# tranqkhue/bugcar_image_segmentation

Measured on AMD Instinct MI355X. Metric: frames/sec ENet 640x480 segmentation -> BEV occupancy grid (synthetic), whole job, higher is better.
Workload: dtype fp32; 1 GPU; config3/5: ENet 640x480 batch 64 per GPU, preprocess + forward + argmax/LUT + fused BEV warp/occgrid (1000x1000 BEV -> 200x200 cells); global_batch=64, per_gpu_batch=64, height=480, width=640, parallelism=frame-sharded dp1, streams_per_gpu=1, hip_graph=True, ranks=1, devices=1, backend=none (one process)

## Files before the change

### bugcar_image_segmentation_amd/build.py

```python
from __future__ import annotations

import os
import subprocess
import sys
from concurrent.futures import ThreadPoolExecutor
from pathlib import Path

PKG = Path(__file__).resolve().parent
ROOT = PKG.parent
CSRC = PKG / "csrc"
OBJ = PKG / "_build"
LIB = PKG / "libbugseg.so"
SOURCES = ["conv_kernels.hip", "cls_kernels.hip", "init_kernels.hip", "bneck_kernels.hip", "bneck2_kernels.hip", "up_kernels.hip", "prep_kernels.hip",
           "bev_kernels.hip", "deeplab_kernels.hip", "road_kernels.hip", "clahe_kernels.hip", "canny_kernels.hip", "eval_kernels.hip", "hough_kernels.hip", "quad_kernels.hip", "bugseg_runtime.cpp", "deeplab_runtime.cpp"]
HEADERS = [CSRC / "bneck_pair_kernels.hip", CSRC / "bugseg_internal.h", CSRC / "deeplab_internal.h", CSRC / "knobs.h", CSRC / "mfma_common.h", CSRC / "cls_common.h", CSRC / "ccl_common.h", ROOT / "include" / "bugseg.h"]
ARCH = os.environ.get("BUGSEG_OFFLOAD_ARCH", "gfx950")
SOURCE_FLAGS = {"cls_kernels.hip": ["-mllvm", "-amdgpu-mfma-vgpr-form=1"], "clahe_kernels.hip": ["-ffp-contract=off"],
                "hough_kernels.hip": ["-ffp-contract=off"], "quad_kernels.hip": ["-ffp-contract=off"]}


def _hipcc() -> str:
    for c in (os.environ.get("HIPCC"), "/opt/rocm/bin/hipcc", "hipcc"):
        if c and (os.path.sep not in c or os.path.exists(c)):
            return c
    raise RuntimeError("hipcc not found")


def _stale(target: Path, deps) -> bool:
    if not target.exists():
        return True
    t = target.stat().st_mtime
    return any(Path(d).stat().st_mtime > t for d in deps)


def build_native(force: bool = False, verbose: bool = False, stamps: bool = False, variant: str = "",
                 defines=()) -> Path:
    if stamps:
        variant, defines = "stamps", ("-DBUGSEG_STAMPS", *defines)
    obj_dir = OBJ / variant if variant else OBJ
    lib = PKG / f"libbugseg_{variant}.so" if variant else LIB
    obj_dir.mkdir(parents=True, exist_ok=True)
    hipcc = _hipcc()
    flags = [f"--offload-arch={ARCH}", "-O3", "-std=c++17", "-fPIC", "-Wall", "-Wno-unused-function",
             f"-I{ROOT / 'include'}", f"-I{CSRC}", *defines]
    jobs = []
    for s in SOURCES:
        src = CSRC / s
        obj = obj_dir / (s + ".o")
        if force or _stale(obj, [src, *HEADERS]):
            lang = ["-x", "hip"] if s.endswith(".hip") else []
            jobs.append((obj, [hipcc, *flags, *SOURCE_FLAGS.get(s, []), *lang, "-c", str(src), "-o", str(obj)]))

    def run(job):
        obj, cmd = job
        if verbose:
            print(" ".join(cmd), file=sys.stderr)
        r = subprocess.run(cmd, capture_output=True, text=True)
        if r.returncode != 0:
            raise RuntimeError(f"compile failed: {' '.join(cmd)}\n{r.stdout}\n{r.stderr}")
        return obj

    with ThreadPoolExecutor(max_workers=min(4, max(1, len(jobs)))) as ex:
        list(ex.map(run, jobs))
    objs = [obj_dir / (s + ".o") for s in SOURCES]
    if force or jobs or _stale(lib, objs):
        tmp = lib.with_suffix(".so.tmp")
        cmd = [hipcc, f"--offload-arch={ARCH}", "-shared", "-fPIC", "-o", str(tmp), *map(str, objs)]
        r = subprocess.run(cmd, capture_output=True, text=True)
        if r.returncode != 0:
            raise RuntimeError(f"link failed: {' '.join(cmd)}\n{r.stdout}\n{r.stderr}")
        os.replace(tmp, lib)
    return lib


if __name__ == "__main__":
    var = next((a.split("=", 1)[1] for a in sys.argv if a.startswith("--variant=")), "")
    print(build_native(force="--force" in sys.argv, verbose=True, stamps="--stamps" in sys.argv, variant=var,
                       defines=tuple(a for a in sys.argv if a.startswith("-D"))))
```

### bugcar_image_segmentation_amd/csrc/bneck_pair_kernels.hip

```cpp
#include <algorithm>

#include "bugseg_internal.h"
#include "mfma_common.h"

namespace bugseg {

namespace {
constexpr int PC = 64, PKS1 = 2, PKS2 = 5, PG2 = 18, PNR3 = 4;
constexpr int PK1S = PKS1 * 32 + 8, PK2S = PKS2 * 32 + 8, PK3S = 32 + 8;
constexpr int PW1 = 16 * PK1S, PW2 = 16 * PK2S, PW3 = PC * PK3S;
constexpr int PWF = PW1 + PW2 + PW3;
constexpr int PCST = 4 * 16 + 3 * PC;
constexpr int PBLK = PWF + PCST;
constexpr int PZP = 8;
#ifndef BNECK_PAIR_YSTR
#define BNECK_PAIR_YSTR 68
#endif
constexpr int PYS = BNECK_PAIR_YSTR;
static_assert(PYS >= PC && PYS % 4 == 0, "a y pixel is 64 floats, 16-B aligned");

template <int TH, int NW>
struct PairForm {
    static constexpr int TW = 16, NT = NW * 64;
    static constexpr int HWA = TW + 4, HRA = (TH + 4) * HWA;
    static constexpr int HWB = TW + 2, HRB = (TH + 2) * HWB;
    static constexpr int NFA = (HRA + 15) / 16, NFB = (HRB + 15) / 16;
    static constexpr int NCA = (NFA + NW - 1) / NW, NCB = (NFB + NW - 1) / NW, NCT = (TH + NW - 1) / NW;
    static constexpr int ZPAD = 2 * PBLK, Y = ZPAD + PZP, T0 = Y + HRB * PYS;
    static constexpr int PLOA = HRA * 8, PLOB = HRB * 8;
    static constexpr int END = T0 + 2 * PLOA;
    static constexpr size_t LDS_BYTES = (size_t)END * 4;
    static_assert(Y % 4 == 0 && T0 % 4 == 0, "every region starts on a 16-B boundary");
    static_assert(NW <= 2 * PLOA, "the range maxima fit in the t0 region");
    static_assert(LDS_BYTES <= 160 * 1024, "a CU has 160 KB of LDS");
};

__device__ __forceinline__ void ldw_hl(RawS &r, const float *p, int kq) {
    r.h = *reinterpret_cast<const uint4 *>(p + kq * 4);
    r.l = *reinterpret_cast<const uint4 *>(p + 16 + kq * 4);
}
__device__ __forceinline__ void st4pl(float *t0, int plo, int h, int ch, float4 v) {
    const float e[4] = {v.x, v.y, v.z, v.w};
    _Float16 hh[4], ll[4];
#pragma unroll
    for (int i = 0; i < 4; ++i) {
        hh[i] = (_Float16)e[i];
        ll[i] = (_Float16)(e[i] - (float)hh[i]);
    }
    unsigned char *b = reinterpret_cast<unsigned char *>(t0 + h * 8) + (ch >> 3) * 16 + (ch & 7) * 2;
    *reinterpret_cast<f16x4 *>(b) = (f16x4){hh[0], hh[1], hh[2], hh[3]};
    *reinterpret_cast<f16x4 *>(b + plo * 4) = (f16x4){ll[0], ll[1], ll[2], ll[3]};
}
}

template <int TH, int NW>
__global__ void __launch_bounds__(NW * 64, 1) bneck_pair_kernel(const BneckPairArgs p) {
    using F = PairForm<TH, NW>;
    constexpr int TW = F::TW, HWA = F::HWA, HRA = F::HRA, HWB = F::HWB, HRB = F::HRB;
    extern __shared__ __attribute__((aligned(16))) float psm[];
    const BneckArgs &a = p.a, &b = p.b;
    span_enter(a.span);
    const int grp = (int)(blockIdx.x & 7), slot = (int)(blockIdx.x >> 3), nslots = (int)(gridDim.x >> 3);
    const int CH = tile_walk_ch(a.ntiles);
    if (tile_walk(grp, slot, CH, a.ntiles, a.rev) < 0) {
        span_exit(a.span);
        return;
    }
    const int tid = threadIdx.x, lane = tid & 63, col = lane & 15, kq = lane >> 4;
    const int wave = __builtin_amdgcn_readfirstlane(tid >> 6);
    const float rl = rng_lane(a.rg);
#pragma unroll
    for (int k = 0; k < 2; ++k) {
        const BneckArgs &q = k ? b : a;
        float *base_k = psm + k * PBLK;
        constexpr int SR1 = PK1S / 4, SR2 = PK2S / 4, SR3 = PK3S / 4, CPR1 = PKS1 * 8, CPR2 = PKS2 * 8, CPR3 = 8;
        constexpr int S1 = 16 * SR1, S2 = 16 * SR2, NSL = PWF / 4;
        static_assert(NSL % 64 == 0, "whole wave instructions");
        for (int base = wave * 64; base < NSL; base += F::NT) {
            const int s = base + lane;
            const uint4 *src;
            auto pick = [&](const void *w, int i, int SR, int CPR) {
                const int r = i / SR, c = i - r * SR;
                const int cs = (c & ~7) | ((c & 7) < 4 ? 2 * (c & 7) : 2 * (c & 3) + 1);
                src = (const uint4 *)w + r * CPR + (c < CPR ? cs : 0);
            };
            if (s < S1) pick(q.w1, s, SR1, CPR1);
            else if (s < S1 + S2) pick(q.w2, s - S1, SR2, CPR2);
            else pick(q.w3, s - S1 - S2, SR3, CPR3);
            __builtin_amdgcn_global_load_lds((__attribute__((address_space(1))) void *)src,
                                             (__attribute__((address_space(3))) void *)(base_k + (size_t)base * 4), 16, 0, 0);
        }
        float *cb1 = base_k + PWF, *cs1 = cb1 + 16, *cb2 = cs1 + 16, *cs2 = cb2 + 16, *cb3 = cs2 + 16, *cs3 = cb3 + PC, *cso = cs3 + PC;
        if (tid < 16) { cb1[tid] = q.b1[tid]; cs1[tid] = q.s1[tid]; cb2[tid] = q.b2[tid]; cs2[tid] = q.s2[tid]; }
        if (tid < PC) { cb3[tid] = q.b3[tid]; cs3[tid] = q.s3[tid]; cso[tid] = q.s_out[tid]; }
    }
    if (tid < PZP) psm[F::ZPAD + tid] = 0.f;
    asm volatile("s_waitcnt vmcnt(0)" ::: "memory");
    if (bneck_range<false>(a.rg, rng_reduce(rl)).any) {
        span_exit(a.span);
        return;
    }
    __syncthreads();

    float *const zpad = psm + F::ZPAD, *const ys = psm + F::Y, *const t0 = psm + F::T0;
    const auto rxb = mkbuf(a.x, a.x_bytes);
    const auto rob = mkbuf(b.out, a.x_bytes);
    auto act = [](float4 v, const float *s) { return prelu4m(v, ld4f(s)); };
    const float4 zero4 = make_float4(0.f, 0.f, 0.f, 0.f);
    float amy = 0.f, amo = 0.f;

    auto blk = [&](int k, const float *&w1, const float *&w2, const float *&w3, const float *&cb1) {
        w1 = psm + k * PBLK; w2 = w1 + PW1; w3 = w2 + PW2; cb1 = w3 + PW3;
    };
    auto project = [&](const float *w1, const float *cb1, const RawF (&xs)[PKS1]) -> float4 {
        f32x4 acc = bias4(cb1 + kq * 4);
#pragma unroll
        for (int s = 0; s < PKS1; ++s) {
            RawS wf;
            ldw_hl(wf, w1 + col * PK1S + s * 32, kq);
            mma(acc, wf, xs[s]);
        }
        return act(f4(acc), cb1 + 16 + kq * 4);
    };
    auto middle = [&](const float *w2, const float *cb2, int hc, int hw, int plo, RawF &tf) {
        f32x4 acc = bias4(cb2 + kq * 4);
#pragma unroll
        for (int s = 0; s < PKS2; ++s) {
            const int g = s * 4 + kq;
            const int tap = g >> 1, coff = (g & 1) * 4;
            const int ky = tap / 3, kx = tap - ky * 3;
            int off = (hc + ky * hw + kx) * 8 + coff;
            asm volatile("" : "+v"(off));
            RawS xf, wf;
            xf.h = *reinterpret_cast<const uint4 *>(g < PG2 ? t0 + off : zpad);
            xf.l = *reinterpret_cast<const uint4 *>(g < PG2 ? t0 + plo + off : zpad);
            ldw_hl(wf, w2 + col * PK2S + s * 32, kq);
            mma(acc, wf, xf);
        }
        to_bop(tf, act(f4(acc), cb2 + 16 + kq * 4), zero4);
    };
    auto expand = [&](const float *w3, const float *cb3, int r, const RawF &tf, float4 res) -> float4 {
        const int ch = r * 16 + kq * 4;
        f32x4 acc = bias4(cb3 + ch);
        RawS wf;
        ldw_hl(wf, w3 + (r * 16 + col) * PK3S, kq);
        mma(acc, wf, tf);
        const float4 v = act(f4(acc), cb3 + PC + ch);
        return act(add4(v, res), cb3 + 2 * PC + ch);
    };

    const int wword = tile_walk_mirror(grp, CH, a.ntiles, a.rev);
    for (int it = slot; it < CH; it += nslots) {
        int tile = grp * CH + it;
        if (tile >= a.ntiles) break;
        tile = tile_walk_flip(wword, tile);
        const int txi = tile % a.tiles_x, t2 = tile / a.tiles_x;
        const int tyi = t2 % a.tiles_y, n = t2 / a.tiles_y;
        const int oy0 = a.oy_base + tyi * TH, ox0 = txi * TW;
        const uint32_t xn = (uint32_t)(n * a.H * a.W) * (uint32_t)(PC * 4);
        auto pix = [&](int y, int x) -> uint32_t {
            uint32_t v = xn + (__umul24((uint32_t)y, (uint32_t)a.W) + (uint32_t)x) * (uint32_t)(PC * 4);
            asm volatile("" : "+v"(v));
            return (unsigned)y < (unsigned)a.H && (unsigned)x < (unsigned)a.W ? v : OOB;
        };
        const float *w1, *w2, *w3, *cb1;

        blk(0, w1, w2, w3, cb1);
        {
            RawF xf[F::NCA][PKS1];
            uint32_t po[F::NCA];
#pragma unroll
            for (int c = 0; c < F::NCA; ++c) {
                const int f = wave + NW * c;
                if (f >= F::NFA) break;
                const int h = f * 16 + col, hy = h / HWA, hx = h - hy * HWA;
                po[c] = h < HRA ? pix(oy0 - 2 + hy, ox0 - 2 + hx) : OOB;
#pragma unroll
                for (int s = 0; s < PKS1; ++s) bld8(xf[c][s], rxb, po[c] == OOB ? OOB : po[c] + (uint32_t)((s * 4 + kq) * 32));
            }
#pragma unroll
            for (int c = 0; c < F::NCA; ++c) {
                const int f = wave + NW * c;
                if (f >= F::NFA) break;
                const int h = f * 16 + col;
                float4 v = project(w1, cb1, xf[c]);
                if (po[c] == OOB) v = zero4;
                if (h < HRA) st4pl(t0, F::PLOA, h, kq * 4, v);
            }
        }
        __syncthreads();

#pragma unroll
        for (int c = 0; c < F::NCB; ++c) {
            const int f = wave + NW * c;
            if (f >= F::NFB) break;
            const int q = f * 16 + col, qq = q < HRB ? q : 0;
            const int ry = qq / HWB, rx = qq - ry * HWB;
            const uint32_t po = q < HRB ? pix(oy0 - 1 + ry, ox0 - 1 + rx) : OOB;
            uint4 res[PNR3];
#pragma unroll
            for (int r = 0; r < PNR3; ++r) res[r] = bld16(rxb, po == OOB ? OOB : po + (uint32_t)((r * 16 + kq * 4) * 4));
            RawF tf;
            middle(w2, cb1 + 32, ry * HWA + rx, HWA, F::PLOA, tf);
#pragma unroll
            for (int r = 0; r < PNR3; ++r) {
                float4 v = expand(w3, cb1 + 64, r, tf, __builtin_bit_cast(float4, res[r]));
                if (po == OOB) v = zero4;
                rng_acc4(amy, v);
                if (q < HRB) st4(ys + q * PYS + r * 16 + kq * 4, v);
            }
        }
        __syncthreads();

        blk(1, w1, w2, w3, cb1);
#pragma unroll
        for (int c = 0; c < F::NCB; ++c) {
            const int f = wave + NW * c;
            if (f >= F::NFB) break;
            const int q = f * 16 + col, qq = q < HRB ? q : 0;
            const int ry = qq / HWB, rx = qq - ry * HWB;
            const bool ok = q < HRB && (unsigned)(oy0 - 1 + ry) < (unsigned)a.H && (unsigned)(ox0 - 1 + rx) < (unsigned)a.W;
            RawF xs[PKS1];
#pragma unroll
            for (int s = 0; s < PKS1; ++s) ld8(xs[s], ys + qq * PYS + (s * 4 + kq) * 8);
            float4 v = project(w1, cb1, xs);
            if (!ok) v = zero4;
            if (q < HRB) st4pl(t0, F::PLOB, q, kq * 4, v);
        }
        __syncthreads();

#pragma unroll
        for (int c = 0; c < F::NCT; ++c) {
            const int f = wave + NW * c;
            if (f >= TH) break;
            RawF tf;
            middle(w2, cb1 + 32, f * HWB + col, HWB, F::PLOB, tf);
            const float *yr = ys + ((f + 1) * HWB + col + 1) * PYS;
            const uint32_t po = pix(oy0 + f, ox0 + col), po_o = pix(oy0 + f, ox0 + (col ^ 8));
            const bool lo8 = col < 8;
            const uint32_t pa = lo8 ? po : po_o, pb = lo8 ? po_o : po;
#pragma unroll
            for (int u = 0; u < PNR3 / 2; ++u) {
                float4 v2[2];
#pragma unroll
                for (int hh = 0; hh < 2; ++hh) {
                    const int r = 2 * u + hh;
                    v2[hh] = expand(w3, cb1 + 64, r, tf, ld4(yr + r * 16 + kq * 4));
                    rng_acc4(amo, v2[hh]);
                }
                const uint4 u0 = __builtin_bit_cast(uint4, v2[0]), u1 = __builtin_bit_cast(uint4, v2[1]);
                const uint4 xs = lo8 ? u1 : u0;
                uint4 yx;
                yx.x = (uint32_t)__builtin_amdgcn_update_dpp(0, (int)xs.x, 0x128, 0xf, 0xf, false);
                yx.y = (uint32_t)__builtin_amdgcn_update_dpp(0, (int)xs.y, 0x128, 0xf, 0xf, false);
                yx.z = (uint32_t)__builtin_amdgcn_update_dpp(0, (int)xs.z, 0x128, 0xf, 0xf, false);
                yx.w = (uint32_t)__builtin_amdgcn_update_dpp(0, (int)xs.w, 0x128, 0xf, 0xf, false);
                const uint32_t cb = (uint32_t)(u * 32 + (lo8 ? 0 : 16) + kq * 4) * 4u;
                bst16o<16>(rob, pa == OOB ? OOB : pa + cb, lo8 ? u0 : yx);
                bst16o<16>(rob, pb == OOB ? OOB : pb + cb, lo8 ? yx : u1);
            }
        }
        __syncthreads();
    }
    rng_commit_wg(amy, a.rg.amax_out, t0, NW);
    rng_commit_wg(amo, b.rg.amax_out, t0, NW);
    span_exit(a.span);
}

#ifndef BNECK_PAIR_TH
#define BNECK_PAIR_TH 12
#endif
#ifndef BNECK_PAIR_NW
#define BNECK_PAIR_NW 16
#endif
using PairBuilt = PairForm<BNECK_PAIR_TH, BNECK_PAIR_NW>;
static const void *pair_fun() { return (const void *)bneck_pair_kernel<BNECK_PAIR_TH, BNECK_PAIR_NW>; }

void bneck_pair_shape(int &th, int &tw, int &threads, size_t &lds) {
    th = BNECK_PAIR_TH; tw = PairBuilt::TW; threads = PairBuilt::NT; lds = PairBuilt::LDS_BYTES;
}

hipError_t launch_bneck_pair(const Knobs &k, const BneckPairArgs &a, hipStream_t s) {
    hipError_t e = allow_dynamic_lds(pair_fun());
    if (e != hipSuccess) return e;
    const int g = resident_grid(k, pair_fun(), PairBuilt::NT, PairBuilt::LDS_BYTES, a.a.ntiles);
    void *args[] = {const_cast<BneckPairArgs *>(&a)};
    return hipLaunchKernel(pair_fun(), dim3(g), dim3(PairBuilt::NT), args, PairBuilt::LDS_BYTES, s);
}

}
```

Baseline: 23560 frames/s.

## Prefetch next tile's input in bneck pair kernel and reuse staged input as residual

```diff
diff --git a/bugcar_image_segmentation_amd/build.py b/bugcar_image_segmentation_amd/build.py
--- a/bugcar_image_segmentation_amd/build.py
+++ b/bugcar_image_segmentation_amd/build.py
@@ -34,9 +34,13 @@
 
 
 def build_native(force: bool = False, verbose: bool = False, stamps: bool = False, variant: str = "",
-                 defines=()) -> Path:
+                 defines=(), only=()) -> Path:
     if stamps:
         variant, defines = "stamps", ("-DBUGSEG_STAMPS", *defines)
+    if not variant:
+        only = ()
+    if only:
+        build_native(verbose=verbose)
     obj_dir = OBJ / variant if variant else OBJ
     lib = PKG / f"libbugseg_{variant}.so" if variant else LIB
     obj_dir.mkdir(parents=True, exist_ok=True)
@@ -45,6 +49,8 @@
              f"-I{ROOT / 'include'}", f"-I{CSRC}", *defines]
     jobs = []
     for s in SOURCES:
+        if only and s not in only:
+            continue
         src = CSRC / s
         obj = obj_dir / (s + ".o")
         if force or _stale(obj, [src, *HEADERS]):
@@ -62,7 +68,7 @@
 
     with ThreadPoolExecutor(max_workers=min(4, max(1, len(jobs)))) as ex:
         list(ex.map(run, jobs))
-    objs = [obj_dir / (s + ".o") for s in SOURCES]
+    objs = [(obj_dir if not only or s in only else OBJ) / (s + ".o") for s in SOURCES]
     if force or jobs or _stale(lib, objs):
         tmp = lib.with_suffix(".so.tmp")
         cmd = [hipcc, f"--offload-arch={ARCH}", "-shared", "-fPIC", "-o", str(tmp), *map(str, objs)]
@@ -75,5 +81,6 @@
 
 if __name__ == "__main__":
     var = next((a.split("=", 1)[1] for a in sys.argv if a.startswith("--variant=")), "")
+    only = next((tuple(a.split("=", 1)[1].split(",")) for a in sys.argv if a.startswith("--only=")), ())
     print(build_native(force="--force" in sys.argv, verbose=True, stamps="--stamps" in sys.argv, variant=var,
-                       defines=tuple(a for a in sys.argv if a.startswith("-D"))))
+                       defines=tuple(a for a in sys.argv if a.startswith("-D")), only=only))
diff --git a/bugcar_image_segmentation_amd/csrc/bneck_pair_kernels.hip b/bugcar_image_segmentation_amd/csrc/bneck_pair_kernels.hip
--- a/bugcar_image_segmentation_amd/csrc/bneck_pair_kernels.hip
+++ b/bugcar_image_segmentation_amd/csrc/bneck_pair_kernels.hip
@@ -18,6 +18,19 @@
 #endif
 constexpr int PYS = BNECK_PAIR_YSTR;
 static_assert(PYS >= PC && PYS % 4 == 0, "a y pixel is 64 floats, 16-B aligned");
+#ifndef BNECK_PAIR_XLDS
+#define BNECK_PAIR_XLDS 1
+#endif
+#ifndef BNECK_PAIR_PREF
+#define BNECK_PAIR_PREF 1
+#endif
+#ifndef BNECK_PAIR_PREFAT
+#define BNECK_PAIR_PREFAT 2
+#endif
+#ifndef STAMP
+#define STAMP(k) do {} while (0)
+#define STAMP_WG() do {} while (0)
+#endif
 
 template <int TH, int NW>
 struct PairForm {
@@ -150,45 +163,76 @@
     };
 
     const int wword = tile_walk_mirror(grp, CH, a.ntiles, a.rev);
-    for (int it = slot; it < CH; it += nslots) {
-        int tile = grp * CH + it;
-        if (tile >= a.ntiles) break;
-        tile = tile_walk_flip(wword, tile);
+    auto tile_at = [&](int it) -> int {
+        const int tile = grp * CH + it;
+        return it < CH && tile < a.ntiles ? tile_walk_flip(wword, tile) : -1;
+    };
+    auto origin = [&](int tile, int &oy0, int &ox0, uint32_t &xn) {
         const int txi = tile % a.tiles_x, t2 = tile / a.tiles_x;
         const int tyi = t2 % a.tiles_y, n = t2 / a.tiles_y;
-        const int oy0 = a.oy_base + tyi * TH, ox0 = txi * TW;
-        const uint32_t xn = (uint32_t)(n * a.H * a.W) * (uint32_t)(PC * 4);
-        auto pix = [&](int y, int x) -> uint32_t {
-            uint32_t v = xn + (__umul24((uint32_t)y, (uint32_t)a.W) + (uint32_t)x) * (uint32_t)(PC * 4);
-            asm volatile("" : "+v"(v));
-            return (unsigned)y < (unsigned)a.H && (unsigned)x < (unsigned)a.W ? v : OOB;
-        };
+        oy0 = a.oy_base + tyi * TH; ox0 = txi * TW;
+        xn = (uint32_t)(n * a.H * a.W) * (uint32_t)(PC * 4);
+    };
+    auto pixn = [&](uint32_t xn, int y, int x) -> uint32_t {
+        uint32_t v = xn + (__umul24((uint32_t)y, (uint32_t)a.W) + (uint32_t)x) * (uint32_t)(PC * 4);
+        asm volatile("" : "+v"(v));
+        return (unsigned)y < (unsigned)a.H && (unsigned)x < (unsigned)a.W ? v : OOB;
+    };
+    constexpr int NPF = BNECK_PAIR_PREF < F::NCA ? BNECK_PAIR_PREF : F::NCA;
+    RawF xf[F::NCA][PKS1];
+    uint32_t pof[F::NCA];
+    auto a1_loads = [&](int tile, int c0, int c1) {
+        int oy0 = 0, ox0 = 0;
+        uint32_t xn = 0;
+        if (tile >= 0) origin(tile, oy0, ox0, xn);
+#pragma unroll
+        for (int c = 0; c < F::NCA; ++c) {
+            const int f = wave + NW * c;
+            if (c < c0 || c >= c1) continue;
+            if (f >= F::NFA) break;
+            const int h = f * 16 + col, hy = h / HWA, hx = h - hy * HWA;
+            pof[c] = h < HRA && tile >= 0 ? pixn(xn, oy0 - 2 + hy, ox0 - 2 + hx) : OOB;
+#pragma unroll
+            for (int s = 0; s < PKS1; ++s) bld8(xf[c][s], rxb, pof[c] == OOB ? OOB : pof[c] + (uint32_t)((s * 4 + kq) * 32));
+        }
+    };
+    if (NPF) a1_loads(tile_at(slot), 0, NPF);
+    for (int it = slot; it < CH; it += nslots) {
+        const int tile = tile_at(it);
+        if (tile < 0) break;
+        int oy0, ox0;
+        uint32_t xn;
+        origin(tile, oy0, ox0, xn);
+        auto pix = [&](int y, int x) -> uint32_t { return pixn(xn, y, x); };
         const float *w1, *w2, *w3, *cb1;
+        STAMP(0); STAMP_WG();
 
         blk(0, w1, w2, w3, cb1);
-        {
-            RawF xf[F::NCA][PKS1];
-            uint32_t po[F::NCA];
-#pragma unroll
-            for (int c = 0; c < F::NCA; ++c) {
-                const int f = wave + NW * c;
-                if (f >= F::NFA) break;
-                const int h = f * 16 + col, hy = h / HWA, hx = h - hy * HWA;
-                po[c] = h < HRA ? pix(oy0 - 2 + hy, ox0 - 2 + hx) : OOB;
-#pragma unroll
-                for (int s = 0; s < PKS1; ++s) bld8(xf[c][s], rxb, po[c] == OOB ? OOB : po[c] + (uint32_t)((s * 4 + kq) * 32));
+        a1_loads(tile, NPF, F::NCA);
+#ifdef BUGSEG_STAMPS
+        asm volatile("s_waitcnt vmcnt(0)" ::: "memory");
+        STAMP(1);
+#endif
+#pragma unroll
+        for (int c = 0; c < F::NCA; ++c) {
+            const int f = wave + NW * c;
+            if (f >= F::NFA) break;
+            const int h = f * 16 + col;
+            if (BNECK_PAIR_XLDS) {
+                const int hy = h / HWA, hx = h - hy * HWA;
+                if (hy >= 1 && hy <= TH + 2 && hx >= 1 && hx <= TW + 2) {
+                    float *xq = ys + ((hy - 1) * HWB + hx - 1) * PYS + kq * 8;
+#pragma unroll
+                    for (int s = 0; s < PKS1; ++s) { st4(xq + s * 32, xf[c][s].a); st4(xq + s * 32 + 4, xf[c][s].b); }
+                }
             }
-#pragma unroll
-            for (int c = 0; c < F::NCA; ++c) {
-                const int f = wave + NW * c;
-                if (f >= F::NFA) break;
-                const int h = f * 16 + col;
-                float4 v = project(w1, cb1, xf[c]);
-                if (po[c] == OOB) v = zero4;
-                if (h < HRA) st4pl(t0, F::PLOA, h, kq * 4, v);
-            }
+            float4 v = project(w1, cb1, xf[c]);
+            if (pof[c] == OOB) v = zero4;
+            if (h < HRA) st4pl(t0, F::PLOA, h, kq * 4, v);
         }
         __syncthreads();
+        STAMP(2);
+        if (NPF && BNECK_PAIR_PREFAT == 2) a1_loads(tile_at(it + nslots), 0, NPF);
 
 #pragma unroll
         for (int c = 0; c < F::NCB; ++c) {
@@ -199,7 +243,9 @@
             const uint32_t po = q < HRB ? pix(oy0 - 1 + ry, ox0 - 1 + rx) : OOB;
             uint4 res[PNR3];
 #pragma unroll
-            for (int r = 0; r < PNR3; ++r) res[r] = bld16(rxb, po == OOB ? OOB : po + (uint32_t)((r * 16 + kq * 4) * 4));
+            for (int r = 0; r < PNR3; ++r)
+                res[r] = BNECK_PAIR_XLDS ? __builtin_bit_cast(uint4, ld4(ys + qq * PYS + r * 16 + kq * 4))
+                                         : bld16(rxb, po == OOB ? OOB : po + (uint32_t)((r * 16 + kq * 4) * 4));
             RawF tf;
             middle(w2, cb1 + 32, ry * HWA + rx, HWA, F::PLOA, tf);
 #pragma unroll
@@ -211,8 +257,10 @@
             }
         }
         __syncthreads();
+        STAMP(3);
 
         blk(1, w1, w2, w3, cb1);
+        if (NPF && BNECK_PAIR_PREFAT == 1) a1_loads(tile_at(it + nslots), 0, NPF);
 #pragma unroll
         for (int c = 0; c < F::NCB; ++c) {
             const int f = wave + NW * c;
@@ -228,6 +276,8 @@
             if (q < HRB) st4pl(t0, F::PLOB, q, kq * 4, v);
         }
         __syncthreads();
+        STAMP(4);
+        if (NPF && BNECK_PAIR_PREFAT == 0) a1_loads(tile_at(it + nslots), 0, NPF);
 
 #pragma unroll
         for (int c = 0; c < F::NCT; ++c) {
@@ -261,6 +311,7 @@
             }
         }
         __syncthreads();
+        STAMP(5);
     }
     rng_commit_wg(amy, a.rg.amax_out, t0, NW);
     rng_commit_wg(amo, b.rg.amax_out, t0, NW);
```

After: 24070 frames/s (median of 6 runs). 1.02x the previous value.
